# srtweezer/RobustGRAPE

Measured on AMD Instinct MI355X. Metric: GRAPE gradient-evals/sec (fidelity+∇), Rydberg CZ d=9 N_t=512, 1→8 GPU, higher is better.
Workload: dtype f64

## Files before the change

robustgrape_amd/csrc/grape_walk_merged.hpp:

```cpp
#pragma once
#include "grape_walk_core.hpp"
#include "grape_walk_gauge.hpp"

namespace grape {

template <int D, bool SMEM>
__device__ __forceinline__ void gauge_prop_lds(const cd *Et, const cd (&e)[kGaugePairs<D>],
                                               MStore<D, false> &E) {
    if constexpr (SMEM) {
        cptr<cd> g = as_constant(Et);
        asm volatile("" : "+s"(g));
#pragma unroll
        for (int j = 0; j < D; ++j) {
#pragma unroll
            for (int k = 0; k < D; ++k) E.set(j, k, gauge_sandwich<D>(e, j, k, cload(g, j * D + k)));
        }
    } else {
#pragma unroll
        for (int j = 0; j < D; ++j) {
#pragma unroll
            for (int k = 0; k < D; ++k) E.set(j, k, gauge_sandwich<D>(e, j, k, Et[j * D + k]));
        }
    }
}
template <int D>
__global__ __launch_bounds__(64) void k_gauge_base_fill(DevProblem P, cd *scr, cd *out, int nsec) {
    const int w = threadIdx.x;
    if (w >= nsec) return;
    WalkX X0;
    X0.k0 = X0.k1 = X0.a0 = X0.a1 = 0.0;
    Pert none;
    none.var = -1;
    none.index = 0;
    none.delta = 0.0;
    SM<D> A[1];
    walk_build<D, 1>(P, as_constant(P.ops) + (size_t)w * P.sec_ops, X0, 1, none, A);
    double mu0 = 0.0;
    walk_expm<D, false, false>(A[0], scr + (size_t)w * 2 * D * D, mu0, true, [&](int i, const cd (&x)[D]) {
#pragma unroll
        for (int j = 0; j < D; ++j) out[(w * D + j) * D + i] = x[j];
    });
}
template <int D, int NE, bool LAD>
__device__ __forceinline__ void merged_step_fwd(const cd *Et, const GaugeN<D> (&gn)[NE], cd p1, cd (&Q)[NE][D][D]) {
#pragma unroll
    for (int w = 0; w < NE; ++w) {
        cd dph[kGaugePairs<D>];
        if constexpr (LAD) gauge_phases_ladder<D>(p1, dph);
        else gauge_phases<D>(p1, gn[w], dph);
        MStore<D, false> E;
        gauge_prop_lds<D, true>(Et + w * D * D, dph, E);
#pragma unroll
        for (int i = 0; i < D; ++i) {
            cd q[D], t[D];
#pragma unroll
            for (int m = 0; m < D; ++m) q[m] = Q[w][m][i];
#pragma unroll
            for (int j = 0; j < D; ++j) {
                cd c = czero();
#pragma unroll
                for (int m = 0; m < D; ++m) cmac(c, q[m], E.at(j, m));
                t[j] = c;
            }
#pragma unroll
            for (int j = 0; j < D; ++j) Q[w][j][i] = t[j];
        }
    }
}
struct WideLane {
    int be, nbe;
    bool ok;
};
__device__ __forceinline__ WideLane wide_lane(const DevBatch &BA) {
    WideLane L;
    const long g = (long)blockIdx.x * kWalkBlock + threadIdx.x;
    L.nbe = BA.nb;
    L.ok = g < (long)L.nbe;
    L.be = L.ok ? (int)g : 0;
    return L;
}
template <int D, int NE, bool LAD>
__device__ __forceinline__ void wide_step_fwd(const cd *Et, const GaugeN<D> (&gn)[NE], cd p1, cd (&psi)[NE][D]) {
#pragma unroll
    for (int w = 0; w < NE; ++w) {
        cd dph[kGaugePairs<D>];
        if constexpr (LAD) gauge_phases_ladder<D>(p1, dph);
        else gauge_phases<D>(p1, gn[w], dph);
        MStore<D, false> E;
        gauge_prop_lds<D, true>(Et + w * D * D, dph, E);
        cd t[D];
#pragma unroll
        for (int j = 0; j < D; ++j) {
            cd c = czero();
#pragma unroll
            for (int m = 0; m < D; ++m) cmac(c, psi[w][m], E.at(j, m));
            t[j] = c;
        }
#pragma unroll
        for (int j = 0; j < D; ++j) psi[w][j] = t[j];
    }
}
template <int D, int NE, int DP>
__device__ __forceinline__ void wide_reframe(const cd (&pw)[DP], cd (&chi)[NE][D]) {
    static_assert(D <= DP, "powers up to the sector's highest charge");
#pragma unroll
    for (int w = 0; w < NE; ++w) {
#pragma unroll
        for (int j = 1; j < D; ++j) chi[w][j] = cmulf(chi[w][j], pw[j]);
    }
}
template <int D, int NE>
__device__ __forceinline__ void wide_step_frame(const cd *Et, cd (&chi)[NE][D]) {
#pragma unroll
    for (int w = 0; w < NE; ++w) {
        cptr<cd> g = as_constant(Et + w * D * D);
        asm volatile("" : "+s"(g));
        cd t[D];
#pragma unroll
        for (int j = 0; j < D; ++j) {
            cd c = czero();
#pragma unroll
            for (int m = 0; m < D; ++m) cmac(c, chi[w][m], cload(g, j * D + m));
            t[j] = c;
        }
#pragma unroll
        for (int j = 0; j < D; ++j) chi[w][j] = t[j];
    }
}
template <int D>
__device__ __forceinline__ void wide_store_psi(cd *u, size_t nbe, const cd (&psi)[D]) {
#pragma unroll
    for (int j = 0; j < D; ++j) u[j * nbe] = psi[j];
}
constexpr int kFdxTile = 16;
__device__ __forceinline__ void wide_load_x(double (*tile)[kFdxTile + 1], const double *x, int nx, int nbe, int j0, int Nt) {
    constexpr int kStep = kWalkBlock / kFdxTile;
    const int j = threadIdx.x % kFdxTile, r0 = threadIdx.x / kFdxTile;
    const double *xc = x + min(j0 + j, Nt - 1);
    const long b0 = (long)blockIdx.x * kWalkBlock;
#pragma unroll 4
    for (int r = r0; r < kWalkBlock; r += kStep) tile[r][j] = xc[(size_t)min(b0 + r, (long)nbe - 1) * nx];
}
__device__ __forceinline__ bool wide_group_full(int nbe) {
    return GRAPE_WIDE_TILE_FAST && ((long)blockIdx.x + 1) * kWalkBlock <= (long)nbe;
}
__device__ __forceinline__ unsigned wide_tile_offset(int nx) {
    return (unsigned)((threadIdx.x / kFdxTile) * nx + threadIdx.x % kFdxTile) * (unsigned)sizeof(double);
}
__device__ __forceinline__ void wide_load_x_full(double (*tile)[kFdxTile + 1], const double *xb, int nx, unsigned off) {
    constexpr int kStep = kWalkBlock / kFdxTile, kTrips = kWalkBlock / kStep;
    const int j = threadIdx.x % kFdxTile, r0 = threadIdx.x / kFdxTile;
    double v[kTrips];
#pragma unroll
    for (int i = 0; i < kTrips; ++i)
        v[i] = *reinterpret_cast<const double *>(reinterpret_cast<const char *>(xb + (size_t)i * kStep * nx) + off);
#pragma unroll
    for (int i = 0; i < kTrips; ++i) tile[r0 + i * kStep][j] = v[i];
}
__device__ __forceinline__ void wide_flush_full(const double (*tile)[kFdxTile + 1], double *fb, int nx, unsigned off) {
    constexpr int kStep = kWalkBlock / kFdxTile, kTrips = kWalkBlock / kStep;
    const int j = threadIdx.x % kFdxTile, r0 = threadIdx.x / kFdxTile;
#pragma unroll
    for (int i = 0; i < kTrips; ++i)
        *reinterpret_cast<double *>(reinterpret_cast<char *>(fb + (size_t)i * kStep * nx) + off) = tile[r0 + i * kStep][j];
}
template <int DA, bool TWB, bool LAD>
__device__ __forceinline__ void wide_fwd_body(const DevProblem &PA, const DevBatch &BA, const DevProblem &PB,
                                              const DevBatch &BB) {
    constexpr int NEB = TWB ? 1 : 2;
    __shared__ double xtile[kWalkBlock][kFdxTile + 1];
    __shared__ grape_cis::CisTabEntry ctab[grape_cis::kCisTabN];
    gauge_cis_stage(ctab);
    const WideLane L = wide_lane(BA);
    GaugeN<DA> gA[1];
    GaugeN<2> gB[NEB];
    gA[0] = gauge_charges<DA>(PA, 0);
#pragma unroll
    for (int w = 0; w < NEB; ++w) gB[w] = gauge_charges<2>(PB, w);
    const int cA = PA.rank1_c[0];
    cd psiA[1][DA], psiB[NEB][2];
#pragma unroll
    for (int j = 0; j < DA; ++j) psiA[0][j] = cmake(j == cA ? 1.0 : 0.0, 0.0);
#pragma unroll
    for (int w = 0; w < NEB; ++w) {
#pragma unroll
        for (int j = 0; j < 2; ++j) psiB[w][j] = cmake(j == PB.rank1_c[w] ? 1.0 : 0.0, 0.0);
    }
    constexpr bool FRAME = LAD && GRAPE_WIDE_STEP_FRAME;
    cd pprev = cmake(1.0, 0.0);
    auto step = [&](double xk) {
        const cd p1 = gauge_cis_tab(PA.gauge_a * xk, ctab);
        if constexpr (FRAME) {
            cd pw[DA];
            ladder_powers<DA>(cmulf(pprev, cconj(p1)), pw);
            pprev = p1;
            wide_reframe<DA, 1>(pw, psiA);
            wide_reframe<2, NEB>(pw, psiB);
            wide_step_frame<DA, 1>(PA.gauge_Et, psiA);
            wide_step_frame<2, NEB>(PB.gauge_Et, psiB);
        } else {
            wide_step_fwd<DA, 1, LAD>(PA.gauge_Et, gA, p1, psiA);
            wide_step_fwd<2, NEB, LAD>(PB.gauge_Et, gB, p1, psiB);
        }
    };
    const bool full = wide_group_full(L.nbe);
    const unsigned off = wide_tile_offset(PA.nx);
    const double *xb = BA.x + (size_t)blockIdx.x * kWalkBlock * PA.nx;
#pragma unroll 1
    for (int j0 = 0; j0 < PA.Nt; j0 += kFdxTile) {
        const int nj = min(kFdxTile, PA.Nt - j0);
        if (full && j0 + kFdxTile <= PA.Nt) wide_load_x_full(xtile, xb + j0, PA.nx, off);
        else wide_load_x(xtile, BA.x, PA.nx, L.nbe, j0, PA.Nt);
        __syncthreads();
        int t = 0;
#pragma unroll 1
        for (; t + 1 < nj; t += 2) {
            step(xtile[threadIdx.x][t]);
            step(xtile[threadIdx.x][t + 1]);
        }
        if (t < nj) step(xtile[threadIdx.x][t]);
        __syncthreads();
    }
    if constexpr (FRAME) {
        cd pw[DA];
        ladder_powers<DA>(pprev, pw);
        wide_reframe<DA, 1>(pw, psiA);
        wide_reframe<2, NEB>(pw, psiB);
    }
    if (L.ok) {
        wide_store_psi<DA>(BA.Ub + L.be, (size_t)L.nbe, psiA[0]);
#pragma unroll
        for (int w = 0; w < NEB; ++w)
            wide_store_psi<2>(BB.Ub + (size_t)w * 2 * L.nbe + L.be, (size_t)L.nbe, psiB[w]);
    }
}
template <int DA, bool TWB, bool LAD, bool WIDE = false>
__global__ __launch_bounds__(kWalkBlock, (WIDE ? GRAPE_WALK_WIDE_FWD_WAVES : GRAPE_WALK_FWD_M_WAVES)) void k_walk_fwd_m(DevProblem PA, DevBatch BA,
                                                                                  DevProblem PB, DevBatch BB) {
    if constexpr (WIDE) {
        wide_fwd_body<DA, TWB, LAD>(PA, BA, PB, BB);
        return;
    }
    constexpr int NEB = TWB ? 1 : 2;
    __shared__ grape_cis::CisTabEntry ctab[grape_cis::kCisTabN];
    gauge_cis_stage(ctab);
    const VBlock vb = hw_block();
    const WalkLane L = walk_lane<1>(PA, BA, vb);
    const double *xt = BA.x + (size_t)L.be * PA.nx;
    const cd *EtA = PA.gauge_Et, *EtB = PB.gauge_Et;
    GaugeN<DA> gA[1];
    GaugeN<2> gB[NEB];
    gA[0] = gauge_charges<DA>(PA, 0);
#pragma unroll
    for (int w = 0; w < NEB; ++w) gB[w] = gauge_charges<2>(PB, w);
    cd QA[1][DA][DA], QB[NEB][2][2];
#pragma unroll
    for (int j = 0; j < DA; ++j) {
#pragma unroll
        for (int i = 0; i < DA; ++i) QA[0][j][i] = cmake(i == j ? 1.0 : 0.0, 0.0);
    }
#pragma unroll
    for (int w = 0; w < NEB; ++w) {
#pragma unroll
        for (int j = 0; j < 2; ++j) {
#pragma unroll
            for (int i = 0; i < 2; ++i) QB[w][j][i] = cmake(i == j ? 1.0 : 0.0, 0.0);
        }
    }
    const int k0 = L.c * PA.L;
    X2 xn = walk_load_x(1, xt + (size_t)min(k0, PA.Nt - 1));
    auto step = [&](int jj) {
        const int k = min(k0 + jj, PA.Nt - 1);
        const double xk = xn.v0;
        xn = walk_load_x(1, xt + (size_t)min(k + 1, PA.Nt - 1));
        const cd p1 = gauge_cis_tab(PA.gauge_a * xk, ctab);
        merged_step_fwd<DA, 1, LAD>(EtA, gA, p1, QA);
        merged_step_fwd<2, NEB, LAD>(EtB, gB, p1, QB);
    };
    const int nlast = PA.Nt - (PA.nchunks - 1) * PA.L;
    int j2 = 0;
#pragma unroll 1
    for (; j2 + 1 < nlast; j2 += 2) {
        step(j2);
        step(j2 + 1);
    }
#pragma unroll 1
    for (; j2 < nlast; ++j2) step(j2);
#pragma unroll 1
    for (int jj = nlast; jj < PA.L; ++jj) {
        if (L.c != PA.nchunks - 1) step(jj);
    }
    if (L.ok) {
        const size_t nbe = (size_t)L.nbe;
        cd *da = BA.Tc + (size_t)L.c * DA * DA * nbe + L.be;
#pragma unroll
        for (int j = 0; j < DA; ++j) {
#pragma unroll
            for (int i = 0; i < DA; ++i) da[(size_t)(j * DA + i) * nbe] = QA[0][j][i];
        }
#pragma unroll
        for (int w = 0; w < NEB; ++w) {
            cd *db = BB.Tc + ((size_t)w * PB.nchunks + L.c) * 4 * nbe + L.be;
#pragma unroll
            for (int j = 0; j < 2; ++j) {
#pragma unroll
                for (int i = 0; i < 2; ++i) db[(size_t)(j * 2 + i) * nbe] = QB[w][j][i];
            }
        }
    }
}
template <int D>
struct SeqChain {
    const cd *T;
    cd *Carry;
    cd P[D][D], tn[D][D];
    __device__ __forceinline__ void init(const cd *T_, cd *Carry_, size_t nbe, size_t be) {
        T = T_ + be;
        Carry = Carry_ + be;
#pragma unroll
        for (int e = 0; e < D * D; ++e) {
            P[e / D][e % D] = cmake(e / D == e % D ? 1.0 : 0.0, 0.0);
            tn[e / D][e % D] = T[(size_t)e * nbe];
        }
    }
    __device__ __forceinline__ void step(int c, int nch, size_t nbe) {
        cd *dc = Carry + (size_t)c * D * D * nbe;
        const cd *tc = T + (size_t)min(c + 1, nch - 1) * D * D * nbe;
        cd t[D][D];
#pragma unroll
        for (int j = 0; j < D; ++j) {
#pragma unroll
            for (int i = 0; i < D; ++i) {
                dc[(size_t)(j * D + i) * nbe] = P[j][i];
                t[j][i] = tn[j][i];
                tn[j][i] = tc[(size_t)(j * D + i) * nbe];
            }
        }
#pragma unroll
        for (int i = 0; i < D; ++i) {
            cd q[D];
#pragma unroll
            for (int m = 0; m < D; ++m) q[m] = P[m][i];
#pragma unroll
            for (int j = 0; j < D; ++j) {
                cd acc = czero();
#pragma unroll
                for (int m = 0; m < D; ++m) cmac(acc, t[j][m], q[m]);
                P[j][i] = acc;
            }
        }
    }
};
constexpr int kSeqBlock = 64;
template <int DA, bool TWB>
__global__ __launch_bounds__(kSeqBlock) void k_scan_seq(DevProblem PA, DevBatch BA, DevProblem PB, DevBatch BB, int nb) {
    constexpr int NEB = TWB ? 1 : 2;
    const size_t be = (size_t)blockIdx.x * kSeqBlock + threadIdx.x;
    if (be >= (size_t)nb) return;
    const size_t nbe = (size_t)nb;
    const int nch = PA.nchunks;
    SeqChain<DA> ca;
    SeqChain<2> cb[NEB];
    ca.init(BA.Tc, BA.Carry, nbe, be);
#pragma unroll
    for (int w = 0; w < NEB; ++w)
        cb[w].init(BB.Tc + (size_t)w * PB.nchunks * 4 * nbe, BB.Carry + (size_t)w * PB.nchunks * 4 * nbe, nbe, be);
#pragma unroll 1
    for (int c = 0; c < nch; ++c) {
        ca.step(c, nch, nbe);
#pragma unroll
        for (int w = 0; w < NEB; ++w) cb[w].step(c, nch, nbe);
    }
    cd *ua = BA.Ub + be * DA * DA;
#pragma unroll
    for (int j = 0; j < DA; ++j) {
#pragma unroll
        for (int i = 0; i < DA; ++i) ua[j * DA + i] = ca.P[j][i];
    }
#pragma unroll
    for (int w = 0; w < NEB; ++w) {
#pragma unroll
        for (int ws = 0; ws < (TWB ? 2 : 1); ++ws) {
            cd *ub = BB.Ub + (be * 2 + w + ws) * 4;
#pragma unroll
            for (int j = 0; j < 2; ++j) {
#pragma unroll
                for (int i = 0; i < 2; ++i) ub[j * 2 + i] = cb[w].P[j][i];
            }
        }
    }
}
template <int D, int NE, int NSEC, bool LAD>
__device__ __forceinline__ double merged_step_grad(const cd *Et, const GaugeN<D> (&gn)[NE], cd p1, cd q,
                                                   double inv_eps, cd (&X)[NSEC][D][D]) {
    constexpr int NSH = NSEC / NE;
    MStore<D, false> E[NE];
#pragma unroll
    for (int w = 0; w < NE; ++w) {
        cd dph[kGaugePairs<D>];
        if constexpr (LAD) gauge_phases_ladder<D>(p1, dph);
        else gauge_phases<D>(p1, gn[w], dph);
        gauge_prop_lds<D, false>(Et + w * D * D, dph, E[w]);
    }
#pragma unroll
    for (int w = 0; w < NSEC; ++w) {
        const int we = w / NSH;
#pragma unroll
        for (int r = 0; r < D; ++r) {
            cd xr[D], y[D];
#pragma unroll
            for (int j = 0; j < D; ++j) xr[j] = X[w][r][j];
#pragma unroll
            for (int cc = 0; cc < D; ++cc) {
                cd s = czero();
#pragma unroll
                for (int j = 0; j < D; ++j) cmac(s, xr[j], cconj(E[we].at(cc, j)));
                y[cc] = s;
            }
#pragma unroll
            for (int cc = 0; cc < D; ++cc) X[w][r][cc] = y[cc];
        }
    }
    double tot = 0.0, one = 0.0;
    if constexpr (LAD && GRAPE_WALK_LADDER_CONTR) {
        cd rh[D];
        ladder_rho<D>(q, rh);
#pragma unroll
        for (int we = 0; we < NE; ++we) {
#pragma unroll
            for (int t = 0; t < NSH; ++t) {
                double tre[D], tim[D];
#pragma unroll
                for (int m = 0; m < D; ++m) tre[m] = tim[m] = 0.0;
#pragma unroll
                for (int r = 0; r < D; ++r) {
#pragma unroll
                    for (int j = 0; j < D; ++j) {
                        if (r == j) continue;
                        const int m = r > j ? r - j : j - r;
                        const cd y = X[we * NSH + t][j][r], e = E[we].at(r, j);
                        tre[m] = fma(y.re, e.re, tre[m]);
                        tre[m] = fma(-y.im, e.im, tre[m]);
                        if (r > j) {
                            tim[m] = fma(y.re, e.im, tim[m]);
                            tim[m] = fma(y.im, e.re, tim[m]);
                        } else {
                            tim[m] = fma(-y.re, e.im, tim[m]);
                            tim[m] = fma(-y.im, e.re, tim[m]);
                        }
                    }
                }
                double c = 0.0;
#pragma unroll
                for (int m = 1; m < D; ++m) {
                    c = fma(rh[m].re, tre[m], c);
                    c = fma(-rh[m].im, tim[m], c);
                }
                const double sv = c * inv_eps;
                tot += sv;
                one = sv;
            }
        }
    } else {
#pragma unroll
    for (int we = 0; we < NE; ++we) {
        double s[NSH];
#pragma unroll
        for (int t = 0; t < NSH; ++t) s[t] = 0.0;
        cd fw[kGaugePairs<D>];
        gauge_fd_weights_dn<D>(q, gn[we], fw);
#pragma unroll
        for (int r = 0; r < D; ++r) {
#pragma unroll
            for (int j = 0; j < D; ++j) {
                if (r == j) continue;
                const cd de = cscale(inv_eps, cmul(E[we].at(r, j), gauge_fd_weight<D>(fw, r, j)));
#pragma unroll
                for (int t = 0; t < NSH; ++t) {
                    const cd y = X[we * NSH + t][j][r];
                    s[t] = fma(y.re, de.re, s[t]);
                    s[t] = fma(-y.im, de.im, s[t]);
                }
            }
        }
#pragma unroll
        for (int t = 0; t < NSH; ++t) {
            tot += s[t];
            one = s[t];
        }
    }
    }
#pragma unroll
    for (int w = 0; w < NSEC; ++w) {
        const int we = w / NSH;
#pragma unroll
        for (int i = 0; i < D; ++i) {
            cd y[D], t[D];
#pragma unroll
            for (int m = 0; m < D; ++m) y[m] = X[w][m][i];
#pragma unroll
            for (int j = 0; j < D; ++j) {
                cd c = czero();
#pragma unroll
                for (int m = 0; m < D; ++m) cmac(c, E[we].at(j, m), y[m]);
                t[j] = c;
            }
#pragma unroll
            for (int j = 0; j < D; ++j) X[w][j][i] = t[j];
        }
    }
    return NSEC > 1 ? tot : one;
}
template <int D, int NE, int NSEC, bool LAD>
__device__ __forceinline__ double merged_step_grad_r1(const cd *Et, const GaugeN<D> (&gn)[NE], cd p1, cd q,
                                                      double inv_eps, cd (&psi)[NSEC][D], cd (&phi)[NSEC][D]) {
    constexpr int NSH = NSEC / NE;
    MStore<D, false> E[NE];
#pragma unroll
    for (int w = 0; w < NE; ++w) {
        cd dph[kGaugePairs<D>];
        if constexpr (LAD) gauge_phases_ladder<D>(p1, dph);
        else gauge_phases<D>(p1, gn[w], dph);
        gauge_prop_lds<D, true>(Et + w * D * D, dph, E[w]);
    }
    cd rh[D];
    if constexpr (LAD) ladder_rho<D>(q, rh);
    double tot = 0.0, one = 0.0;
#pragma unroll
    for (int we = 0; we < NE; ++we) {
        cd fw[kGaugePairs<D>];
        if constexpr (!LAD) {
            gauge_fd_weights_dn<D>(q, gn[we], fw);
        }
#pragma unroll
        for (int t = 0; t < NSH; ++t) {
            const int w = we * NSH + t;
            cd f[D], u[D][D];
#pragma unroll
            for (int r = 0; r < D; ++r) {
                cd c = czero();
#pragma unroll
                for (int j = 0; j < D; ++j) cmac(c, E[we].at(r, j), phi[w][j]);
                f[r] = c;
            }
#pragma unroll
            for (int r = 0; r < D; ++r) {
                phi[w][r] = f[r];
#pragma unroll
                for (int j = 0; j < D; ++j) u[r][j] = cmulf(E[we].at(r, j), psi[w][j]);
            }
            double c = 0.0;
            if constexpr (LAD) {
                double tre[D], tim[D];
#pragma unroll
                for (int m = 0; m < D; ++m) tre[m] = tim[m] = 0.0;
#pragma unroll
                for (int r = 0; r < D; ++r) {
#pragma unroll
                    for (int j = 0; j < D; ++j) {
                        if (r == j) continue;
                        const int m = r > j ? r - j : j - r;
                        tre[m] = fma(f[r].re, u[r][j].re, tre[m]);
                        tre[m] = fma(f[r].im, u[r][j].im, tre[m]);
                        if (r > j) {
                            tim[m] = fma(f[r].re, u[r][j].im, tim[m]);
                            tim[m] = fma(-f[r].im, u[r][j].re, tim[m]);
                        } else {
                            tim[m] = fma(-f[r].re, u[r][j].im, tim[m]);
                            tim[m] = fma(f[r].im, u[r][j].re, tim[m]);
                        }
                    }
                }
#pragma unroll
                for (int m = 1; m < D; ++m) {
                    c = fma(rh[m].re, tre[m], c);
                    c = fma(-rh[m].im, tim[m], c);
                }
            } else {
#pragma unroll
                for (int r = 0; r < D; ++r) {
#pragma unroll
                    for (int j = 0; j < D; ++j) {
                        if (r == j) continue;
                        const cd z = cmulf(cconj(f[r]), u[r][j]), g = gauge_fd_weight<D>(fw, r, j);
                        c = fma(z.re, g.re, c);
                        c = fma(-z.im, g.im, c);
                    }
                }
            }
            const double sv = c * inv_eps;
            tot += sv;
            one = sv;
#pragma unroll
            for (int r = 0; r < D; ++r) {
                cd s = u[r][0];
#pragma unroll
                for (int j = 1; j < D; ++j) s = cadd(s, u[r][j]);
                psi[w][r] = s;
            }
        }
    }
    return NSEC > 1 ? tot : one;
}
template <int D>
__device__ __forceinline__ void merged_r1_init(const cd *ca, size_t nbe, const cd *Mw, const cd *Mw2, int c,
                                               cd (&psi)[D], cd (&phi)[D]) {
    cd m[D];
#pragma unroll
    for (int e = 0; e < D; ++e) m[e] = cconj(Mw2 ? cadd(Mw[c * D + e], Mw2[c * D + e]) : Mw[c * D + e]);
#pragma unroll
    for (int j = 0; j < D; ++j) {
        cd s = czero();
#pragma unroll
        for (int e = 0; e < D; ++e) cmac(s, ca[(size_t)(j * D + e) * nbe], m[e]);
        phi[j] = s;
        psi[j] = ca[(size_t)(j * D + c) * nbe];
    }
}
template <int D, int NE, int NSEC, bool LAD, int DR>
__device__ __forceinline__ double wide_step_grad(const cd *Et, const GaugeN<D> (&gn)[NE], cd p1, const cd (&rh)[DR],
                                                 const cd (&fw)[NE][kGaugePairs<D>], double inv_eps,
                                                 cd (&psi)[NSEC][D], cd (&phi)[NSEC][D]) {
    static_assert(D <= DR, "weights up to the sector's highest charge difference");
    constexpr int NSH = NSEC / NE;
    MStore<D, false> E[NE];
#pragma unroll
    for (int w = 0; w < NE; ++w) {
        cd dph[kGaugePairs<D>];
        if constexpr (LAD) gauge_phases_ladder<D>(p1, dph);
        else gauge_phases<D>(p1, gn[w], dph);
        gauge_prop_lds<D, true>(Et + w * D * D, dph, E[w]);
    }
    double tot = 0.0, one = 0.0;
#pragma unroll
    for (int we = 0; we < NE; ++we) {
#pragma unroll
        for (int t = 0; t < NSH; ++t) {
            const int w = we * NSH + t;
            cd pm[D], v[D][D];
#pragma unroll
            for (int j = 0; j < D; ++j) {
                cd s = czero();
#pragma unroll
                for (int r = 0; r < D; ++r) cmac(s, cconj(E[we].at(r, j)), psi[w][r]);
                pm[j] = s;
            }
#pragma unroll
            for (int r = 0; r < D; ++r) {
#pragma unroll
                for (int j = 0; j < D; ++j) v[r][j] = cmulf(cconj(phi[w][r]), E[we].at(r, j));
            }
            double c = 0.0;
            if constexpr (LAD) {
                double tre[D], tim[D];
#pragma unroll
                for (int m = 0; m < D; ++m) tre[m] = tim[m] = 0.0;
#pragma unroll
                for (int r = 0; r < D; ++r) {
#pragma unroll
                    for (int j = 0; j < D; ++j) {
                        if (r == j) continue;
                        const int m = r > j ? r - j : j - r;
                        tre[m] = fma(v[r][j].re, pm[j].re, tre[m]);
                        tre[m] = fma(-v[r][j].im, pm[j].im, tre[m]);
                        if (r > j) {
                            tim[m] = fma(v[r][j].re, pm[j].im, tim[m]);
                            tim[m] = fma(v[r][j].im, pm[j].re, tim[m]);
                        } else {
                            tim[m] = fma(-v[r][j].re, pm[j].im, tim[m]);
                            tim[m] = fma(-v[r][j].im, pm[j].re, tim[m]);
                        }
                    }
                }
#pragma unroll
                for (int m = 1; m < D; ++m) {
                    c = fma(rh[m].re, tre[m], c);
                    c = fma(-rh[m].im, tim[m], c);
                }
            } else {
#pragma unroll
                for (int r = 0; r < D; ++r) {
#pragma unroll
                    for (int j = 0; j < D; ++j) {
                        if (r == j) continue;
                        const cd z = cmulf(v[r][j], pm[j]), g = gauge_fd_weight<D>(fw[we], r, j);
                        c = fma(z.re, g.re, c);
                        c = fma(-z.im, g.im, c);
                    }
                }
            }
            const double sv = c * inv_eps;
            tot += sv;
            one = sv;
#pragma unroll
            for (int j = 0; j < D; ++j) {
                cd s = v[0][j];
#pragma unroll
                for (int r = 1; r < D; ++r) s = cadd(s, v[r][j]);
                phi[w][j] = cconj(s);
                psi[w][j] = pm[j];
            }
        }
    }
    return NSEC > 1 ? tot : one;
}
__device__ __forceinline__ double wide_uniform(double v) {
    const int lo = __builtin_amdgcn_readfirstlane(__double2loint(v)), hi = __builtin_amdgcn_readfirstlane(__double2hiint(v));
    return __hiloint2double(hi, lo);
}
template <int DA, int NEB, bool LAD>
struct WideFd {
    static constexpr int NW = LAD ? DA - 1 : kGaugePairs<DA> + NEB;
    double eps, thr;
    grape_fd::Base b[NW];
};
template <int DA, int NEB, bool LAD>
__device__ __forceinline__ void wide_fd_base(double a, double eps, const GaugeN<DA> (&gA)[1], const GaugeN<2> (&gB)[NEB],
                                             WideFd<DA, NEB, LAD> &fd) {
    static_assert(DA >= 2, "class B's pair reads rho(1)");
    const cd q0 = cis_m1(a * eps);
    int mmax = 0;
    auto take = [&](int i, cd f, int dn) {
        const grape_fd::Base b = grape_fd::fd_base_h(grape_fd::fd_base_signed(grape_fd::Z{f.re, f.im}, dn), a);
        fd.b[i].rho0 = grape_fd::Z{wide_uniform(b.rho0.re), wide_uniform(b.rho0.im)};
        fd.b[i].g = (LAD && NEB == 1) ? b.g : grape_fd::Z{wide_uniform(b.g.re), wide_uniform(b.g.im)};
        mmax = max(mmax, dn < 0 ? -dn : dn);
    };
    if constexpr (LAD) {
        cd rh0[DA];
        ladder_rho<DA>(q0, rh0);
#pragma unroll
        for (int m = 1; m < DA; ++m) take(m - 1, rh0[m], m);
    } else {
        cd f0[kGaugePairs<DA>], f1[1];
        gauge_fd_weights_dn<DA>(q0, gA[0], f0);
#pragma unroll
        for (int r = 0; r < DA; ++r) {
#pragma unroll
            for (int j = r + 1; j < DA; ++j) take(gauge_pair(DA, r, j), f0[gauge_pair(DA, r, j)], gA[0].n[r] - gA[0].n[j]);
        }
#pragma unroll
        for (int w = 0; w < NEB; ++w) {
            gauge_fd_weights_dn<2>(q0, gB[w], f1);
            take(kGaugePairs<DA> + w, f1[0], gB[w].n[0] - gB[w].n[1]);
        }
    }
    fd.eps = eps;
    fd.thr = wide_uniform(grape_fd::fd_threshold_h(a, eps, mmax));
}
template <int DA, int NEB, bool LAD>
__device__ __forceinline__ void wide_fd_weights(const WideFd<DA, NEB, LAD> &fd, double a, double h, const GaugeN<DA> (&gA)[1],
                                                const GaugeN<2> (&gB)[NEB], cd (&rh)[DA], cd (&fwA)[1][kGaugePairs<DA>],
                                                cd (&fwB)[NEB][1]) {
    const double dh = h - fd.eps;
    auto at = [&](int i) {
        const grape_fd::Z z = grape_fd::fd_step(fd.b[i], dh);
        return cmake(z.re, z.im);
    };
    if (fabs(dh) <= fd.thr) {
        if constexpr (LAD) {
            rh[0] = czero();
#pragma unroll
            for (int m = 1; m < DA; ++m) rh[m] = at(m - 1);
        } else {
#pragma unroll
            for (int i = 0; i < kGaugePairs<DA>; ++i) fwA[0][i] = at(i);
#pragma unroll
            for (int w = 0; w < NEB; ++w) fwB[w][0] = at(kGaugePairs<DA> + w);
        }
    } else {
        const cd q = cis_m1(a * h);
        if constexpr (LAD) {
            ladder_rho<DA>(q, rh);
        } else {
            gauge_fd_weights_dn<DA>(q, gA[0], fwA[0]);
#pragma unroll
            for (int w = 0; w < NEB; ++w) gauge_fd_weights_dn<2>(q, gB[w], fwB[w]);
        }
    }
}
template <int D>
__device__ __forceinline__ void wide_grad_init(const cd *u, size_t nbe, const cd *a, const cd *a2, int c, cd (&psi)[D],
                                               cd (&phi)[D]) {
    const cd al = cconj(a2 ? cadd(*a, *a2) : *a);
#pragma unroll
    for (int j = 0; j < D; ++j) {
        psi[j] = u[j * nbe];
        phi[j] = j == c ? al : czero();
    }
}
template <int DA, bool TWB, bool LAD>
__device__ __forceinline__ void wide_grad_body(const DevProblem &PA, const DevBatch &BA, const DevProblem &PB,
                                               const DevBatch &BB, double (*ftile)[kFdxTile + 1], int2 *frow,
                                               const grape_cis::CisTabEntry *ctab) {
    constexpr int NEB = TWB ? 1 : 2;
    constexpr int NXB = (TWB && GRAPE_WALK_TWIN_SUM) ? 1 : 2;
    const WideLane L = wide_lane(BA);
    frow[threadIdx.x] = make_int2(L.ok ? L.be : -1, 0);
    cd psiA[1][DA], phiA[1][DA], psiB[NXB][2], phiB[NXB][2];
    const size_t be = (size_t)L.be;
    const size_t nbe = (size_t)L.nbe;
    wide_grad_init<DA>(BA.Ub + be, nbe, BA.Msec + be, nullptr, PA.rank1_c[0], psiA[0], phiA[0]);
#pragma unroll
    for (int w = 0; w < NXB; ++w) {
        const cd *ab = BB.Msec + be * 2 + w;
        wide_grad_init<2>(BB.Ub + (size_t)(TWB ? 0 : w) * 2 * nbe + be, nbe, ab, NXB == 1 ? ab + 1 : nullptr, PB.rank1_c[w],
                          psiB[w], phiB[w]);
    }
    GaugeN<DA> gA[1];
    GaugeN<2> gB[NEB];
    gA[0] = gauge_charges<DA>(PA, 0);
#pragma unroll
    for (int w = 0; w < NEB; ++w) gB[w] = gauge_charges<2>(PB, w);
    WideFd<DA, NEB, LAD> fd;
    wide_fd_base<DA, NEB, LAD>(PA.gauge_a, PA.eps, gA, gB, fd);
    auto step = [&](double xk) {
        const double xe = xk + PA.eps;
        const cd p1 = gauge_cis_tab(PA.gauge_a * xk, ctab);
        cd rh[DA], fwA[1][kGaugePairs<DA>], fwB[NEB][1];
        wide_fd_weights<DA, NEB, LAD>(fd, PA.gauge_a, xe - xk, gA, gB, rh, fwA, fwB);
        const double sa = wide_step_grad<DA, 1, 1, LAD>(PA.gauge_Et, gA, p1, rh, fwA, PA.inv_eps, psiA, phiA);
        const double sb = wide_step_grad<2, NEB, NXB, LAD>(PB.gauge_Et, gB, p1, rh, fwB, PB.inv_eps, psiB, phiB);
        return sa + sb;
    };
    const int jlast = (PA.Nt - 1) / kFdxTile * kFdxTile;
    const bool full = wide_group_full(L.nbe);
    const unsigned off = wide_tile_offset(PA.nx);
    const size_t row0 = (size_t)blockIdx.x * kWalkBlock * PA.nx;
#pragma unroll 1
    for (int j0 = jlast; j0 >= 0; j0 -= kFdxTile) {
        const int nj = min(kFdxTile, PA.Nt - j0);
        const bool fast = full && j0 + kFdxTile <= PA.Nt;
        if (fast) wide_load_x_full(ftile, BA.x + row0 + j0, PA.nx, off);
        else wide_load_x(ftile, BA.x, PA.nx, L.nbe, j0, PA.Nt);
        __syncthreads();
#pragma unroll 1
        for (int t = nj - 1; t >= 0; --t) ftile[threadIdx.x][t] = step(ftile[threadIdx.x][t]);
        __syncthreads();
        if (fast) {
            wide_flush_full(ftile, BA.Fdx + row0 + j0, PA.nx, off);
        } else {
            const int j = threadIdx.x % kFdxTile;
#pragma unroll 1
            for (int row = threadIdx.x / kFdxTile; row < kWalkBlock; row += kWalkBlock / kFdxTile) {
                const int br = frow[row].x;
                if (j < nj && br >= 0) BA.Fdx[(size_t)br * PA.nx + j0 + j] = ftile[row][j];
            }
        }
        __syncthreads();
    }
}
template <int DA, bool TWB, bool LAD, bool R1, bool WIDE = false>
__global__ __launch_bounds__(kWalkBlock, (WIDE ? GRAPE_WALK_WIDE_GRAD_WAVES : R1 ? GRAPE_WALK_R1_WAVES : GRAPE_WALK_MERGED_WAVES)) void k_walk_grad_m(DevProblem PA, DevBatch BA,
                                                                                   DevProblem PB, DevBatch BB) {
    constexpr int NEB = TWB ? 1 : 2;
    __shared__ double ftile[kWalkBlock][kFdxTile + 1];
    __shared__ int2 frow[kWalkBlock];
    __shared__ grape_cis::CisTabEntry ctab[grape_cis::kCisTabN];
    gauge_cis_stage(ctab);
    if constexpr (WIDE) {
        wide_grad_body<DA, TWB, LAD>(PA, BA, PB, BB, ftile, frow, ctab);
        return;
    }
    const VBlock vb = hw_block();
    const WalkLane L = walk_lane<1>(PA, BA, vb);
    const double *xt = BA.x + (size_t)L.be * PA.nx;
    frow[threadIdx.x] = make_int2(L.ok ? L.be : -1, L.c * PA.L);
    constexpr int NXB = (TWB && GRAPE_WALK_TWIN_SUM) ? 1 : 2;
    cd XA[1][DA][DA], XB[NXB][2][2];
    cd psiA[1][DA], phiA[1][DA], psiB[NXB][2], phiB[NXB][2];
    if constexpr (R1) {
        const size_t nbe = (size_t)L.nbe, be = (size_t)L.be;
        merged_r1_init<DA>(BA.Carry + (size_t)L.c * DA * DA * nbe + be, nbe, BA.Msec + be * DA * DA, nullptr, PA.rank1_c[0],
                           psiA[0], phiA[0]);
#pragma unroll
        for (int w = 0; w < NXB; ++w) {
            const cd *mb = BB.Msec + (be * 2 + w) * 4;
            merged_r1_init<2>(BB.Carry + ((size_t)(TWB ? 0 : w) * PB.nchunks + L.c) * 4 * nbe + be, nbe, mb,
                              NXB == 1 ? mb + 4 : nullptr, PB.rank1_c[w], psiB[w], phiB[w]);
        }
    } else {
        const size_t nbe = (size_t)L.nbe, be = (size_t)L.be;
        cd Cr[DA * DA];
        const cd *ca = BA.Carry + (size_t)L.c * DA * DA * nbe + be;
#pragma unroll
        for (int e = 0; e < DA * DA; ++e) Cr[e] = ca[(size_t)e * nbe];
        merged_xinit<DA>(Cr, BA.Msec + be * DA * DA, XA[0]);
#pragma unroll
        for (int w = 0; w < NXB; ++w) {
            cd Cb[4], Mb[4];
            const cd *cb = BB.Carry + ((size_t)(TWB ? 0 : w) * PB.nchunks + L.c) * 4 * nbe + be;
            const cd *mb = BB.Msec + (be * 2 + w) * 4;
#pragma unroll
            for (int e = 0; e < 4; ++e) {
                Cb[e] = cb[(size_t)e * nbe];
                Mb[e] = NXB == 1 ? cadd(mb[e], mb[4 + e]) : mb[e];
            }
            merged_xinit<2>(Cb, Mb, XB[w]);
        }
    }
    const cd *EtA = R1 ? PA.gauge_Et
                       : gauge_base_lds<DA, 1>(PA, as_constant(PA.ops), BA.wscr + (size_t)L.slot * 2 * DA * DA);
    const cd *EtB = R1 ? PB.gauge_Et
                       : gauge_base_lds<2, NEB>(PB, as_constant(PB.ops), BB.wscr + (size_t)L.slot * 2 * 2 * 4);
    GaugeN<DA> gA[1];
    GaugeN<2> gB[NEB];
    gA[0] = gauge_charges<DA>(PA, 0);
#pragma unroll
    for (int w = 0; w < NEB; ++w) gB[w] = gauge_charges<2>(PB, w);
    const int k0 = L.c * PA.L;
    X2 xn = walk_load_x(1, xt + (size_t)min(k0, PA.Nt - 1));
    auto step = [&](int jj) {
        const int k = min(k0 + jj, PA.Nt - 1);
        const double xk = xn.v0, xe = xk + PA.eps;
        xn = walk_load_x(1, xt + (size_t)min(k + 1, PA.Nt - 1));
        const cd p1 = gauge_cis_tab(PA.gauge_a * xk, ctab), q = cis_m1(PA.gauge_a * (xe - xk));
        double sa, sb;
        if constexpr (R1) {
            sa = merged_step_grad_r1<DA, 1, 1, LAD>(EtA, gA, p1, q, PA.inv_eps, psiA, phiA);
            sb = merged_step_grad_r1<2, NEB, NXB, LAD>(EtB, gB, p1, q, PB.inv_eps, psiB, phiB);
        } else {
            sa = merged_step_grad<DA, 1, 1, LAD>(EtA, gA, p1, q, PA.inv_eps, XA);
            sb = merged_step_grad<2, NEB, NXB, LAD>(EtB, gB, p1, q, PB.inv_eps, XB);
        }
        return sa + sb;
    };
#pragma unroll 1
    for (int j0 = 0; j0 < PA.L; j0 += kFdxTile) {
        const int nj = min(kFdxTile, PA.L - j0);
#pragma unroll 1
        for (int t = 0; t < nj; ++t) ftile[threadIdx.x][t] = step(j0 + t);
        __syncthreads();
        const int j = threadIdx.x % kFdxTile;
#pragma unroll 1
        for (int row = threadIdx.x / kFdxTile; row < kWalkBlock; row += kWalkBlock / kFdxTile) {
            const int br = frow[row].x, kk = frow[row].y + j0 + j;
            if (j < nj && br >= 0 && kk < PA.Nt) BA.Fdx[(size_t)br * PA.nx + kk] = ftile[row][j];
        }
        __syncthreads();
    }
}

}
```

Measured before the change: 141.1 million.

## Use rotating-frame ladder steps in wide backward gradient walk

```diff
diff --git a/robustgrape_amd/csrc/grape_walk_merged.hpp b/robustgrape_amd/csrc/grape_walk_merged.hpp
--- a/robustgrape_amd/csrc/grape_walk_merged.hpp
+++ b/robustgrape_amd/csrc/grape_walk_merged.hpp
@@ -187,18 +187,18 @@
         for (int j = 0; j < 2; ++j) psiB[w][j] = cmake(j == PB.rank1_c[w] ? 1.0 : 0.0, 0.0);
     }
     constexpr bool FRAME = LAD && GRAPE_WIDE_STEP_FRAME;
-    cd pprev = cmake(1.0, 0.0);
+    double xprev = 0.0;
     auto step = [&](double xk) {
-        const cd p1 = gauge_cis_tab(PA.gauge_a * xk, ctab);
         if constexpr (FRAME) {
             cd pw[DA];
-            ladder_powers<DA>(cmulf(pprev, cconj(p1)), pw);
-            pprev = p1;
+            ladder_powers<DA>(gauge_cis_tab(PA.gauge_a * (xprev - xk), ctab), pw);
+            xprev = xk;
             wide_reframe<DA, 1>(pw, psiA);
             wide_reframe<2, NEB>(pw, psiB);
             wide_step_frame<DA, 1>(PA.gauge_Et, psiA);
             wide_step_frame<2, NEB>(PB.gauge_Et, psiB);
         } else {
+            const cd p1 = gauge_cis_tab(PA.gauge_a * xk, ctab);
             wide_step_fwd<DA, 1, LAD>(PA.gauge_Et, gA, p1, psiA);
             wide_step_fwd<2, NEB, LAD>(PB.gauge_Et, gB, p1, psiB);
         }
@@ -223,7 +223,7 @@
     }
     if constexpr (FRAME) {
         cd pw[DA];
-        ladder_powers<DA>(pprev, pw);
+        ladder_powers<DA>(gauge_cis_tab(PA.gauge_a * xprev, ctab), pw);
         wide_reframe<DA, 1>(pw, psiA);
         wide_reframe<2, NEB>(pw, psiB);
     }
@@ -617,18 +617,16 @@
         psi[j] = ca[(size_t)(j * D + c) * nbe];
     }
 }
-template <int D, int NE, int NSEC, bool LAD, int DR>
-__device__ __forceinline__ double wide_step_grad(const cd *Et, const GaugeN<D> (&gn)[NE], cd p1, const cd (&rh)[DR],
+template <int D, int NE, int NSEC>
+__device__ __forceinline__ double wide_step_grad(const cd *Et, const GaugeN<D> (&gn)[NE], cd p1,
                                                  const cd (&fw)[NE][kGaugePairs<D>], double inv_eps,
                                                  cd (&psi)[NSEC][D], cd (&phi)[NSEC][D]) {
-    static_assert(D <= DR, "weights up to the sector's highest charge difference");
     constexpr int NSH = NSEC / NE;
     MStore<D, false> E[NE];
 #pragma unroll
     for (int w = 0; w < NE; ++w) {
         cd dph[kGaugePairs<D>];
-        if constexpr (LAD) gauge_phases_ladder<D>(p1, dph);
-        else gauge_phases<D>(p1, gn[w], dph);
+        gauge_phases<D>(p1, gn[w], dph);
         gauge_prop_lds<D, true>(Et + w * D * D, dph, E[w]);
     }
     double tot = 0.0, one = 0.0;
@@ -651,42 +649,14 @@
                 for (int j = 0; j < D; ++j) v[r][j] = cmulf(cconj(phi[w][r]), E[we].at(r, j));
             }
             double c = 0.0;
-            if constexpr (LAD) {
-                double tre[D], tim[D];
-#pragma unroll
-                for (int m = 0; m < D; ++m) tre[m] = tim[m] = 0.0;
-#pragma unroll
-                for (int r = 0; r < D; ++r) {
-#pragma unroll
-                    for (int j = 0; j < D; ++j) {
-                        if (r == j) continue;
-                        const int m = r > j ? r - j : j - r;
-                        tre[m] = fma(v[r][j].re, pm[j].re, tre[m]);
-                        tre[m] = fma(-v[r][j].im, pm[j].im, tre[m]);
-                        if (r > j) {
-                            tim[m] = fma(v[r][j].re, pm[j].im, tim[m]);
-                            tim[m] = fma(v[r][j].im, pm[j].re, tim[m]);
-                        } else {
-                            tim[m] = fma(-v[r][j].re, pm[j].im, tim[m]);
-                            tim[m] = fma(-v[r][j].im, pm[j].re, tim[m]);
-                        }
-                    }
-                }
-#pragma unroll
-                for (int m = 1; m < D; ++m) {
-                    c = fma(rh[m].re, tre[m], c);
-                    c = fma(-rh[m].im, tim[m], c);
-                }
-            } else {
-#pragma unroll
-                for (int r = 0; r < D; ++r) {
-#pragma unroll
-                    for (int j = 0; j < D; ++j) {
-                        if (r == j) continue;
-                        const cd z = cmulf(v[r][j], pm[j]), g = gauge_fd_weight<D>(fw[we], r, j);
-                        c = fma(z.re, g.re, c);
-                        c = fma(-z.im, g.im, c);
-                    }
+#pragma unroll
+            for (int r = 0; r < D; ++r) {
+#pragma unroll
+                for (int j = 0; j < D; ++j) {
+                    if (r == j) continue;
+                    const cd z = cmulf(v[r][j], pm[j]), g = gauge_fd_weight<D>(fw[we], r, j);
+                    c = fma(z.re, g.re, c);
+                    c = fma(-z.im, g.im, c);
                 }
             }
             const double sv = c * inv_eps;
@@ -699,6 +669,73 @@
                 for (int r = 1; r < D; ++r) s = cadd(s, v[r][j]);
                 phi[w][j] = cconj(s);
                 psi[w][j] = pm[j];
+            }
+        }
+    }
+    return NSEC > 1 ? tot : one;
+}
+template <int D, int NE, int NSEC, int DR>
+__device__ __forceinline__ double wide_step_grad_frame(const cd *Et, const cd (&rh)[DR], double inv_eps,
+                                                       cd (&chi)[NSEC][D], cd (&eta)[NSEC][D]) {
+    static_assert(D <= DR, "weights up to the sector's highest charge difference");
+    constexpr int NSH = NSEC / NE;
+    double tot = 0.0, one = 0.0;
+#pragma unroll
+    for (int we = 0; we < NE; ++we) {
+        cptr<cd> g = as_constant(Et + we * D * D);
+        asm volatile("" : "+s"(g));
+#pragma unroll
+        for (int t = 0; t < NSH; ++t) {
+            const int w = we * NSH + t;
+            cd pm[D], v[D][D];
+#pragma unroll
+            for (int j = 0; j < D; ++j) {
+                cd s = czero();
+#pragma unroll
+                for (int r = 0; r < D; ++r) cmac(s, cconj(cload(g, r * D + j)), chi[w][r]);
+                pm[j] = s;
+            }
+#pragma unroll
+            for (int r = 0; r < D; ++r) {
+#pragma unroll
+                for (int j = 0; j < D; ++j) v[r][j] = cmulf(cconj(eta[w][r]), cload(g, r * D + j));
+            }
+            double tre[D], tim[D];
+#pragma unroll
+            for (int m = 0; m < D; ++m) tre[m] = tim[m] = 0.0;
+#pragma unroll
+            for (int r = 0; r < D; ++r) {
+#pragma unroll
+                for (int j = 0; j < D; ++j) {
+                    if (r == j) continue;
+                    const int m = r > j ? r - j : j - r;
+                    tre[m] = fma(v[r][j].re, pm[j].re, tre[m]);
+                    tre[m] = fma(-v[r][j].im, pm[j].im, tre[m]);
+                    if (r > j) {
+                        tim[m] = fma(v[r][j].re, pm[j].im, tim[m]);
+                        tim[m] = fma(v[r][j].im, pm[j].re, tim[m]);
+                    } else {
+                        tim[m] = fma(-v[r][j].re, pm[j].im, tim[m]);
+                        tim[m] = fma(-v[r][j].im, pm[j].re, tim[m]);
+                    }
+                }
+            }
+            double c = 0.0;
+#pragma unroll
+            for (int m = 1; m < D; ++m) {
+                c = fma(rh[m].re, tre[m], c);
+                c = fma(-rh[m].im, tim[m], c);
+            }
+            const double sv = c * inv_eps;
+            tot += sv;
+            one = sv;
+#pragma unroll
+            for (int j = 0; j < D; ++j) {
+                cd s = v[0][j];
+#pragma unroll
+                for (int r = 1; r < D; ++r) s = cadd(s, v[r][j]);
+                eta[w][j] = cconj(s);
+                chi[w][j] = pm[j];
             }
         }
     }
@@ -814,14 +851,29 @@
     for (int w = 0; w < NEB; ++w) gB[w] = gauge_charges<2>(PB, w);
     WideFd<DA, NEB, LAD> fd;
     wide_fd_base<DA, NEB, LAD>(PA.gauge_a, PA.eps, gA, gB, fd);
+    double xlast = 0.0;
     auto step = [&](double xk) {
         const double xe = xk + PA.eps;
-        const cd p1 = gauge_cis_tab(PA.gauge_a * xk, ctab);
         cd rh[DA], fwA[1][kGaugePairs<DA>], fwB[NEB][1];
-        wide_fd_weights<DA, NEB, LAD>(fd, PA.gauge_a, xe - xk, gA, gB, rh, fwA, fwB);
-        const double sa = wide_step_grad<DA, 1, 1, LAD>(PA.gauge_Et, gA, p1, rh, fwA, PA.inv_eps, psiA, phiA);
-        const double sb = wide_step_grad<2, NEB, NXB, LAD>(PB.gauge_Et, gB, p1, rh, fwB, PB.inv_eps, psiB, phiB);
-        return sa + sb;
+        if constexpr (LAD) {
+            cd pw[DA];
+            ladder_powers<DA>(gauge_cis_tab(PA.gauge_a * (xlast - xk), ctab), pw);
+            xlast = xk;
+            wide_fd_weights<DA, NEB, LAD>(fd, PA.gauge_a, xe - xk, gA, gB, rh, fwA, fwB);
+            wide_reframe<DA, 1>(pw, psiA);
+            wide_reframe<DA, 1>(pw, phiA);
+            wide_reframe<2, NXB>(pw, psiB);
+            wide_reframe<2, NXB>(pw, phiB);
+            const double sa = wide_step_grad_frame<DA, 1, 1>(PA.gauge_Et, rh, PA.inv_eps, psiA, phiA);
+            const double sb = wide_step_grad_frame<2, NEB, NXB>(PB.gauge_Et, rh, PB.inv_eps, psiB, phiB);
+            return sa + sb;
+        } else {
+            const cd p1 = gauge_cis_tab(PA.gauge_a * xk, ctab);
+            wide_fd_weights<DA, NEB, LAD>(fd, PA.gauge_a, xe - xk, gA, gB, rh, fwA, fwB);
+            const double sa = wide_step_grad<DA, 1, 1>(PA.gauge_Et, gA, p1, fwA, PA.inv_eps, psiA, phiA);
+            const double sb = wide_step_grad<2, NEB, NXB>(PB.gauge_Et, gB, p1, fwB, PB.inv_eps, psiB, phiB);
+            return sa + sb;
+        }
     };
     const int jlast = (PA.Nt - 1) / kFdxTile * kFdxTile;
     const bool full = wide_group_full(L.nbe);
```

New measurement: 148.3 million, median of 6. 1.05x the previous value.
